# likojack/bnv_fusion

Hardware: AMD Instinct MI355X
Metric: depth frames/sec fused+decoded, 640x480 @ 256^3 grid (higher is better)
Workload: dtype f32 operands split into f16 hi+lo, 3 products on v_mfma_f32_16x16x32_f16, f32 accumulate

## Files before the change

### bnv_fusion_amd/csrc/encode_mlp.hip

```cpp
#include "encode.hpp"

namespace bnv {

__device__ __forceinline__ f32x16 relu16(f32x16 v) {
#pragma unroll
  for (int r = 0; r < 16; ++r) v[r] = relu_bits(v[r]);
  return v;
}

__device__ __forceinline__ f32x16 bias_init(const float* __restrict__ b, int mb, int h) {
  f32x16 v;
#pragma unroll
  for (int q = 0; q < 4; ++q) {
    const f32x4 t = *(const f32x4*)&b[mb * 32 + 8 * q + 4 * h];
#pragma unroll
    for (int i = 0; i < 4; ++i) v[4 * q + i] = t[i];
  }
  return v;
}

__device__ __forceinline__ void layer128(const float* __restrict__ wp, const float* __restrict__ bias,
                                         const f32x16 (&in)[4], f32x16 (&out)[4], int lane, int h) {
#pragma unroll
  for (int mb = 0; mb < 4; ++mb) out[mb] = bias_init(bias, mb, h);
#pragma unroll
  for (int nb = 0; nb < 4; ++nb) {
#pragma unroll
    for (int rq = 0; rq < 4; ++rq) {
      f32x4 a[4];
#pragma unroll
      for (int mb = 0; mb < 4; ++mb)
        a[mb] = *(const f32x4*)&wp[(((mb * 4 + nb) * 4 + rq) * 64 + lane) * 4];
#pragma unroll
      for (int i = 0; i < 4; ++i) {
#pragma unroll
        for (int mb = 0; mb < 4; ++mb)
          out[mb] = __builtin_amdgcn_mfma_f32_32x32x2f32(a[mb][i], in[nb][4 * rq + i], out[mb], 0, 0, 0);
      }
    }
  }
}

__global__ __launch_bounds__(512, 2) void k_pointnet_scatter(
    const float* __restrict__ pts, int n_points, bnv_grid_t g, const float* __restrict__ wpack,
    const uint32_t* __restrict__ bitmap, const uint32_t* __restrict__ word_prefix,
    int32_t* __restrict__ counts, long long* __restrict__ acc, const int32_t* __restrict__ pair_list,
    const int32_t* __restrict__ n_pairs) {
  extern __shared__ __attribute__((aligned(16))) float lds[];
  stage_to_lds<512>(wpack, lds, PN_TOTAL * 4);
  __syncthreads();

  const int lane = threadIdx.x & 63;
  const int wave = __builtin_amdgcn_readfirstlane(threadIdx.x >> 6);
  const int j = lane & 31, h = lane >> 5;
  const PairTiles T = pair_tiles(n_points, pair_list, n_pairs);
  const int n_tiles = T.n_tiles;

  for (int t = blockIdx.x * 8 + wave; t < n_tiles; t += gridDim.x * 8) {
    int i = 0, k = 0;
    const bool have = tile_pair(T, t, j, &i, &k);
    float in0 = 0.f, in1 = 0.f, in2 = 0.f;
    int slot = -1;
    bool valid = false;
    if (have) {
      const float* p = pts + (size_t)i * 6;
      const float x = p[0], y = p[1], z = p[2];
      valid = in_bounds(x, y, z, g);
      if (valid) {
        const float xn = voxel_coord(x, g.bound_min[0], g.voxel_size);
        const float yn = voxel_coord(y, g.bound_min[1], g.voxel_size);
        const float zn = voxel_coord(z, g.bound_min[2], g.voxel_size);
        int gx, gy, gz;
        const uint32_t id = corner_voxel(k, xn, yn, zn, g, gx, gy, gz);
        if (voxel_owner(gx, gy, gz, g) == g.shard_rank) slot = slot_rank(bitmap[id >> 5], word_prefix[id >> 5], id);
        const float rx = relative_coord(xn, gx, g.voxel_size);
        const float ry = relative_coord(yn, gy, g.voxel_size);
        const float rz = relative_coord(zn, gz, g.voxel_size);
        in0 = h ? ry : rx;
        in1 = h ? p[3] : rz;
        in2 = h ? p[5] : p[4];
      }
    }
    if (__ballot(slot >= 0) == 0ULL) continue;

    f32x16 ha[4], hb[4];
#pragma unroll
    for (int mb = 0; mb < 4; ++mb) ha[mb] = bias_init(lds + PN_B1, mb, h);
    {
      const float bin[3] = {in0, in1, in2};
#pragma unroll
      for (int s = 0; s < 3; ++s) {
#pragma unroll
        for (int mb = 0; mb < 4; ++mb)
          ha[mb] = __builtin_amdgcn_mfma_f32_32x32x2f32(lds[PN_W1 + (s * 4 + mb) * 64 + lane], bin[s],
                                                        ha[mb], 0, 0, 0);
      }
    }
#pragma unroll
    for (int mb = 0; mb < 4; ++mb) ha[mb] = relu16(ha[mb]);
    layer128(lds + PN_W2, lds + PN_B2, ha, hb, lane, h);
#pragma unroll
    for (int mb = 0; mb < 4; ++mb) hb[mb] = relu16(hb[mb]);
    layer128(lds + PN_W3, lds + PN_B3, hb, ha, lane, h);
#pragma unroll
    for (int mb = 0; mb < 4; ++mb) ha[mb] = relu16(ha[mb]);
    f32x16 o;
#pragma unroll
    for (int r = 0; r < 16; ++r) o[r] = 0.f;
    {
      const f32x4 b4 = *(const f32x4*)&lds[PN_B4 + 4 * h];
#pragma unroll
      for (int r = 0; r < 4; ++r) o[r] = b4[r];
    }
#pragma unroll
    for (int nb = 0; nb < 4; ++nb) {
#pragma unroll
      for (int rq = 0; rq < 4; ++rq) {
        f32x4 a = {0.f, 0.f, 0.f, 0.f};
        if (j < 8) a = *(const f32x4*)&lds[PN_W4 + ((((nb * 4 + rq) * 2 + h) * 8) + j) * 4];
#pragma unroll
        for (int i = 0; i < 4; ++i)
          o = __builtin_amdgcn_mfma_f32_32x32x2f32(a[i], ha[nb][4 * rq + i], o, 0, 0, 0);
      }
    }
    scatter_tile(o, slot, j, h, counts, acc);
  }
}

typedef __attribute__((address_space(3))) const half8 lds_half8_t;
typedef __attribute__((address_space(3))) const f32x4 lds_f32x4_t;
constexpr int kLdsWin = 61440;

#ifdef BNV_PHASE_PROF
__device__ unsigned long long g_enc_phase[8 * 16];
#define BNV_EPH(i)                                                                          \
  do {                                                                                      \
    if ((threadIdx.x & 63) == 0) {                                                          \
      unsigned long long* _p = (unsigned long long*)((char*)lds + PX_LDS_BYTES) + (threadIdx.x >> 6) * 16; \
      const unsigned long long _t = clock64();                                              \
      _p[i] += _t - _p[15];                                                                 \
      _p[15] = _t;                                                                          \
    }                                                                                       \
  } while (0)
constexpr int kEncProfLds = 8 * 16 * 8;
#else
#define BNV_EPH(i)
constexpr int kEncProfLds = 0;
#endif

struct EncLdsX {
  uint32_t w[3];
  uint32_t b;
};
__device__ __forceinline__ half8 ldsx_wfrag(const EncLdsX& L, int byte_off) {
  const int b = byte_off / kLdsWin;
  return *(lds_half8_t*)((b == 0 ? L.w[0] : (b == 1 ? L.w[1] : L.w[2])) + (uint32_t)(byte_off - b * kLdsWin));
}
__device__ __forceinline__ f32x4 ldsx_bias(const EncLdsX& L, int layer, int rb) {
  return *(lds_f32x4_t*)(L.b + (uint32_t)((layer * 128 + rb * 16) * 4));
}

template <int NPROD>
__device__ __forceinline__ void layer128_x(const EncLdsX& L, int w_off, int layer, const half8 (&inh)[4][2],
                                           const half8 (&inl)[4][2], f32x4 (&out)[8][2]) {
#pragma unroll
  for (int rb = 0; rb < 8; ++rb) out[rb][0] = out[rb][1] = ldsx_bias(L, layer, rb);
  half8 ah[2], al[2];
#define BNV_LOAD_WX(q)                                                        \
  {                                                                           \
    const int wb = (w_off + (q) * 2 * 64 * 8) * 2;                            \
    ah[(q) & 1] = ldsx_wfrag(L, wb);                                          \
    if (NPROD == 3) al[(q) & 1] = ldsx_wfrag(L, wb + 1024);                   \
  }
  BNV_LOAD_WX(0);
#pragma unroll
  for (int q = 0; q < 32; ++q) {
    if (q + 1 < 32) BNV_LOAD_WX(q + 1);
    __builtin_amdgcn_sched_barrier(0);
    const int s = q >> 3, rb = q & 7;
    if constexpr (NPROD == 3) {
      out[rb][0] = __builtin_amdgcn_mfma_f32_16x16x32_f16(al[q & 1], inh[s][0], out[rb][0], 0, 0, 0);
      out[rb][1] = __builtin_amdgcn_mfma_f32_16x16x32_f16(al[q & 1], inh[s][1], out[rb][1], 0, 0, 0);
      out[rb][0] = __builtin_amdgcn_mfma_f32_16x16x32_f16(ah[q & 1], inl[s][0], out[rb][0], 0, 0, 0);
      out[rb][1] = __builtin_amdgcn_mfma_f32_16x16x32_f16(ah[q & 1], inl[s][1], out[rb][1], 0, 0, 0);
    }
    out[rb][0] = __builtin_amdgcn_mfma_f32_16x16x32_f16(ah[q & 1], inh[s][0], out[rb][0], 0, 0, 0);
    out[rb][1] = __builtin_amdgcn_mfma_f32_16x16x32_f16(ah[q & 1], inh[s][1], out[rb][1], 0, 0, 0);
    __builtin_amdgcn_sched_barrier(0);
  }
#undef BNV_LOAD_WX
}

template <int NPROD>
__device__ __forceinline__ void split_x(const f32x4 (&acc)[8][2], half8 (&oh)[4][2], half8 (&ol)[4][2]) {
#pragma unroll
  for (int s = 0; s < 4; ++s)
#pragma unroll
    for (int cb = 0; cb < 2; ++cb) {
      float x[8];
#pragma unroll
      for (int e = 0; e < 8; ++e) x[e] = relu_bits(acc[2 * s + (e >> 2)][cb][e & 3]);
      if (NPROD == 3) {
        split8_f16(x, oh[s][cb], ol[s][cb]);
      } else {
#pragma unroll
        for (int e = 0; e < 8; ++e) oh[s][cb][e] = (_Float16)x[e];
      }
    }
}

__device__ __forceinline__ void scatter_tile_x(const f32x4& o, int slot, int n, int g, int32_t* __restrict__ counts,
                                               long long* __restrict__ acc) {
  uint32_t lo[4], hi[4];
#pragma unroll
  for (int q = 0; q < 4; ++q) fixed_hi_lo(o[q], hi[q], lo[q]);
  asm volatile(BNV_SCAN_ROWS : BNV_SCAN_REGS(lo, hi) : : "vcc");
  {
    const int tsrc = ((g & 1) * 16 + 15) * 4;
#pragma unroll
    for (int q = 0; q < 4; ++q) {
      const uint32_t tl = (uint32_t)__builtin_amdgcn_ds_bpermute(tsrc, (int)lo[q]);
      const uint32_t th = (uint32_t)__builtin_amdgcn_ds_bpermute(tsrc, (int)hi[q]);
      if (g >= 2) {
        const unsigned long long v = (((unsigned long long)hi[q] << 32) | lo[q]) + (((unsigned long long)th << 32) | tl);
        lo[q] = (uint32_t)v;
        hi[q] = (uint32_t)(v >> 32);
      }
    }
  }
  const int p = (g >> 1) * 16 + n;
  const int slot15 = __builtin_amdgcn_readlane(slot, 15);
  const int prev_row = __builtin_amdgcn_update_dpp(0, slot, 0x111 , 0xf, 0xf, false);
  const int prev = n == 0 ? slot15 : prev_row;
  const unsigned long long heads64 = __ballot(p == 0 || prev != slot);
  const uint32_t heads = ((uint32_t)heads64 & 0xffffu) | (((uint32_t)(heads64 >> 32) & 0xffffu) << 16);
  const int s = 31 - __clz((int)(heads & (0xffffffffu >> (31 - p))));
  const bool is_end = p == 31 || ((heads >> (p + 1)) & 1u);
  const int sp = s > 0 ? s - 1 : 0;
  const int src = (((sp >> 4) * 2 + (g & 1)) * 16 + (sp & 15)) * 4;
  uint32_t plo[4], phi[4];
#pragma unroll
  for (int q = 0; q < 4; ++q) {
    plo[q] = (uint32_t)__builtin_amdgcn_ds_bpermute(src, (int)lo[q]);
    phi[q] = (uint32_t)__builtin_amdgcn_ds_bpermute(src, (int)hi[q]);
  }
#ifdef BNV_PROBE_NO_SCATTER
  if ((blockIdx.x & 63) != 0) return;
#endif
  if (slot >= 0 && is_end) {
    unsigned long long* dst = (unsigned long long*)acc + ((uint32_t)slot * 8u + 4u * (uint32_t)(g & 1));
#pragma unroll
    for (int q = 0; q < 4; ++q) {
      unsigned long long v = ((unsigned long long)hi[q] << 32) | lo[q];
      if (s > 0) v -= ((unsigned long long)phi[q] << 32) | plo[q];
      atomicAdd(dst + q, v);
    }
    if ((g & 1) == 0) atomicAdd(&counts[slot], p - s + 1);
  }
}

template <int NPROD>
__global__ __launch_bounds__(512, 2) __attribute__((amdgpu_num_vgpr(120))) void k_pointnet_scatter_x(
    const float* __restrict__ pts, int n_points, bnv_grid_t g, const float* __restrict__ wpack,
    const uint32_t* __restrict__ bitmap, const uint32_t* __restrict__ word_prefix,
    int32_t* __restrict__ counts, long long* __restrict__ acc, int32_t* __restrict__ error,
    const int32_t* __restrict__ pair_list, const int32_t* __restrict__ n_pairs) {
  extern __shared__ __attribute__((aligned(16))) float lds[];
  const float n_cert = wpack[PN_CERT];
  float* lb = lds + PX_TOTAL / 2;
  for (int i = threadIdx.x; i < 128 * 3 + 8; i += 512) lb[i] = wpack[PN_B1 + i];
  stage_to_lds<512>(wpack + PX_OFF, lds, PX_TOTAL * 2);
  int* tile_ctr = (int*)((char*)lds + PX_TOTAL * 2 + (128 * 3 + 8) * 4);
  if (threadIdx.x == 0) *tile_ctr = 0;
  __syncthreads();

  const int lane = threadIdx.x & 63;
  const int n = lane & 15, gk = lane >> 4;
  const int pair = (gk >> 1) * 16 + n;
  const PairTiles T = pair_tiles(n_points, pair_list, n_pairs);
  const int n_tiles = T.n_tiles;
  const int nyz = g.n_xyz[1] * g.n_xyz[2];
  EncLdsX L;
  {
    const uint32_t lds0 = (uint32_t)(uintptr_t)(__attribute__((address_space(3))) float*)lds;
    L.w[0] = lds0 + lane * 16;
    L.w[1] = L.w[0] + kLdsWin;
    L.w[2] = L.w[0] + 2 * kLdsWin;
    L.b = lds0 + PX_TOTAL * 2 + gk * 16;
    asm volatile("" : "+v"(L.w[0]), "+v"(L.w[1]), "+v"(L.w[2]), "+v"(L.b));
  }

  const int tstep = gridDim.x * 8;
  auto grab = [&]() -> int {
    int c = 0;
    if (lane == 0) c = atomicAdd(tile_ctr, 1);
    c = __builtin_amdgcn_readfirstlane(c);
    return blockIdx.x * 8 + (c & 7) + (c >> 3) * tstep;
  };
  float raw[6];
  int raw_k = 0;
  bool raw_ok = false;
  float nin[6];
  uint32_t n_id = 0, n_word = 0, n_pref = 0;
  bool n_own = false;
  auto stage1 = [&](int t) {
    raw_ok = false;
    if (t < n_tiles) {
      int i = 0;
      if (tile_pair(T, t, pair, &i, &raw_k)) {
        const float* p = pts + (size_t)i * 6;
#pragma unroll
        for (int c = 0; c < 6; ++c) raw[c] = p[c];
        raw_ok = true;
      }
    }
  };
  auto stage2 = [&](int t) {
    n_own = false;
#pragma unroll
    for (int c = 0; c < 6; ++c) nin[c] = 0.f;
    if (raw_ok && in_bounds(raw[0], raw[1], raw[2], g)) {
      const int k = raw_k;
      const float xn = voxel_coord(raw[0], g.bound_min[0], g.voxel_size);
      const float yn = voxel_coord(raw[1], g.bound_min[1], g.voxel_size);
      const float zn = voxel_coord(raw[2], g.bound_min[2], g.voxel_size);
      int gx, gy, gz;
      corner_xyz(k, xn, yn, zn, gx, gy, gz);
      if (voxel_owner(gx, gy, gz, g) == g.shard_rank) {
        n_own = true;
        n_id = voxel_id(gx, gy, gz, nyz, g.n_xyz[2]);
        n_word = bitmap[n_id >> 5];
        n_pref = word_prefix[n_id >> 5];
      }
      if ((gk & 1) == 0) {
        nin[0] = relative_coord(xn, gx, g.voxel_size);
        nin[1] = relative_coord(yn, gy, g.voxel_size);
        nin[2] = relative_coord(zn, gz, g.voxel_size);
        nin[3] = raw[3];
        nin[4] = raw[4];
        nin[5] = raw[5];
      }
      if (!(fmaxf(fmaxf(fabsf(raw[3]), fabsf(raw[4])), fabsf(raw[5])) <= n_cert)) *error = 3;
    }
  };
  int t = grab();
  stage1(t);
  stage2(t);
  int t_next = grab(), t_next2 = 0;
  stage1(t_next);
#ifdef BNV_PHASE_PROF
  if ((threadIdx.x & 63) < 16)
    ((unsigned long long*)((char*)lds + PX_LDS_BYTES))[(threadIdx.x >> 6) * 16 + (threadIdx.x & 63)] = 0;
  if ((threadIdx.x & 63) == 0) ((unsigned long long*)((char*)lds + PX_LDS_BYTES))[(threadIdx.x >> 6) * 16 + 15] = clock64();
#endif

  for (; t < n_tiles; t = t_next, t_next = t_next2) {
    float in[6];
#pragma unroll
    for (int c = 0; c < 6; ++c) in[c] = nin[c];
    const int slot = n_own ? slot_rank(n_word, n_pref, n_id) : -1;
    stage2(t_next);
    t_next2 = grab();
    stage1(t_next2);
    __builtin_amdgcn_sched_barrier(0);
    BNV_EPH(0);
    if (__ballot(slot >= 0) == 0ULL) continue;

    f32x4 ha[8][2], hb[8][2];
    {
      half8 bh[2], bl[2];
#pragma unroll
      for (int cb = 0; cb < 2; ++cb) {
        float x[8];
#pragma unroll
        for (int e = 0; e < 8; ++e) x[e] = 0.f;
#pragma unroll
        for (int e = 0; e < 6; ++e) {
          const float other = __shfl(in[e], (lane + 32) & 63, 64);
          x[e] = gk == 0 ? (cb == 0 ? in[e] : other) : 0.f;
        }
        if (NPROD == 3) {
          split8_f16(x, bh[cb], bl[cb]);
        } else {
#pragma unroll
          for (int e = 0; e < 8; ++e) bh[cb][e] = (_Float16)x[e];
        }
      }
#pragma unroll
      for (int rb = 0; rb < 8; ++rb) {
        const half8 ahi = ldsx_wfrag(L, (PX_W1 + rb * 2 * 64 * 8) * 2), alo = ldsx_wfrag(L, (PX_W1 + rb * 2 * 64 * 8) * 2 + 1024);
        const f32x4 b = ldsx_bias(L, 0, rb);
#pragma unroll
        for (int cb = 0; cb < 2; ++cb) {
          f32x4 c = b;
          if constexpr (NPROD == 3) {
            c = __builtin_amdgcn_mfma_f32_16x16x32_f16(alo, bh[cb], c, 0, 0, 0);
            c = __builtin_amdgcn_mfma_f32_16x16x32_f16(ahi, bl[cb], c, 0, 0, 0);
          }
          ha[rb][cb] = __builtin_amdgcn_mfma_f32_16x16x32_f16(ahi, bh[cb], c, 0, 0, 0);
        }
      }
    }
    BNV_EPH(1);
    half8 sh[4][2], sl[4][2];
    split_x<NPROD>(ha, sh, sl);
    BNV_EPH(2);
    layer128_x<NPROD>(L, PX_W2, 1, sh, sl, hb);
    BNV_EPH(3);
    split_x<NPROD>(hb, sh, sl);
    BNV_EPH(4);
    layer128_x<NPROD>(L, PX_W3, 2, sh, sl, ha);
    BNV_EPH(5);
    split_x<NPROD>(ha, sh, sl);
    BNV_EPH(6);
    f32x4 o[2];
    o[0] = o[1] = *(lds_f32x4_t*)(L.b + 384 * 4);
    {
      half8 w4h[4], w4l[4];
      __builtin_amdgcn_sched_barrier(0);
#pragma unroll
      for (int s = 0; s < 4; ++s) {
        w4h[s] = ldsx_wfrag(L, (PX_W4 + s * 2 * 64 * 8) * 2);
        if (NPROD == 3) w4l[s] = ldsx_wfrag(L, (PX_W4 + s * 2 * 64 * 8) * 2 + 1024);
      }
#pragma unroll
      for (int s = 0; s < 4; ++s) {
#pragma unroll
        for (int cb = 0; cb < 2; ++cb) {
          if constexpr (NPROD == 3) {
            o[cb] = __builtin_amdgcn_mfma_f32_16x16x32_f16(w4l[s], sh[s][cb], o[cb], 0, 0, 0);
            o[cb] = __builtin_amdgcn_mfma_f32_16x16x32_f16(w4h[s], sl[s][cb], o[cb], 0, 0, 0);
          }
          o[cb] = __builtin_amdgcn_mfma_f32_16x16x32_f16(w4h[s], sh[s][cb], o[cb], 0, 0, 0);
        }
      }
    }
    f32x4 mine;
#pragma unroll
    for (int i = 0; i < 4; ++i) {
      const float other = __shfl(o[1][i], (lane + 32) & 63, 64);
      mine[i] = gk < 2 ? o[0][i] : other;
    }
    BNV_EPH(7);
    scatter_tile_x(mine, slot, n, gk, counts, acc);
    BNV_EPH(8);
  }
#ifdef BNV_PHASE_PROF
  if ((threadIdx.x & 63) < 15)
    atomicAdd(&g_enc_phase[(threadIdx.x >> 6) * 16 + (threadIdx.x & 63)],
              ((unsigned long long*)((char*)lds + PX_LDS_BYTES))[(threadIdx.x >> 6) * 16 + (threadIdx.x & 63)]);
#endif
}

int encode_init() {
  const hipFuncAttribute lds = hipFuncAttributeMaxDynamicSharedMemorySize;
  BNV_HIP_CHECK(hipFuncSetAttribute((const void*)k_pointnet_scatter, lds, PN_TOTAL * 4));
  BNV_HIP_CHECK(hipFuncSetAttribute((const void*)k_pointnet_scatter_x<3>, lds, PX_LDS_BYTES + kEncProfLds));
  BNV_HIP_CHECK(hipFuncSetAttribute((const void*)k_pointnet_scatter_x<1>, lds, PX_LDS_BYTES + kEncProfLds));
  return BNV_OK;
}

void launch_encoder_mlp(int mlp, int grid, const float* pts, int n, const bnv_grid_t& g, const float* pack,
                        const EncodeWs& ws, const int32_t* plist, hipStream_t stream) {
  if (mlp == 1 || mlp == 3)
    hipLaunchKernelGGL(mlp == 1 ? k_pointnet_scatter_x<3> : k_pointnet_scatter_x<1>, dim3(grid), dim3(512),
                       PX_LDS_BYTES + kEncProfLds, stream, pts, n, g, pack, ws.bitmap, ws.word_prefix, ws.counts,
                       ws.acc, &ws.ctl->error, plist, &ws.ctl->n_pairs);
  else
    hipLaunchKernelGGL(k_pointnet_scatter, dim3(grid), dim3(512), PN_TOTAL * 4, stream, pts, n, g, pack, ws.bitmap,
                       ws.word_prefix, ws.counts, ws.acc, plist, &ws.ctl->n_pairs);
}

}

#ifdef BNV_PHASE_PROF
extern "C" int bnv_dev_enc_phase_read(unsigned long long* out128) {
  BNV_HIP_CHECK(hipDeviceSynchronize());
  BNV_HIP_CHECK(hipMemcpyFromSymbol(out128, HIP_SYMBOL(bnv::g_enc_phase), 128 * sizeof(unsigned long long)));
  unsigned long long z[128] = {};
  BNV_HIP_CHECK(hipMemcpyToSymbol(HIP_SYMBOL(bnv::g_enc_phase), z, sizeof(z)));
  return BNV_OK;
}
#endif
```

### bnv_fusion_amd/weights.py

```python
import os

import numpy as np

_HERE = os.path.dirname(os.path.abspath(__file__))
DEFAULT_FP32 = os.path.join(_HERE, "weights", "pointnet_fp32.npz")
DEFAULT_TCNN = os.path.join(_HERE, "weights", "pointnet_tcnn.npz")

BN_EPS = 1e-5


def load_npz(path=DEFAULT_FP32):
    with np.load(path) as z:
        return {k: z[k] for k in z.files}


def _np(v):
    return v.detach().cpu().numpy() if hasattr(v, "detach") else np.asarray(v)


def fold_pointnet(sd):
    out = []
    for i in (1, 2, 3, 4):
        p = "pointnet_backbone."
        W = _np(sd[f"{p}conv{i}.weight"]).astype(np.float64)[:, :, 0]
        b = _np(sd[f"{p}conv{i}.bias"]).astype(np.float64)
        s = _np(sd[f"{p}bn{i}.weight"]).astype(np.float64) / np.sqrt(
            _np(sd[f"{p}bn{i}.running_var"]).astype(np.float64) + BN_EPS)
        Wf = W * s[:, None]
        bf = (b - _np(sd[f"{p}bn{i}.running_mean"]).astype(np.float64)) * s + _np(sd[f"{p}bn{i}.bias"]).astype(
            np.float64)
        out.append((Wf.astype(np.float32), bf.astype(np.float32)))
    return out


F16_MAX = 65504.0


def certified_input_bound(layers, fixed, n_free, limit=0.98 * F16_MAX):
    W0 = np.abs(np.asarray(layers[0][0], dtype=np.float64))
    fixed = np.asarray(fixed, dtype=np.float64)
    k = len(fixed)
    assert W0.shape[1] == k + n_free
    a = W0[:, :k] @ fixed + np.abs(np.asarray(layers[0][1], dtype=np.float64))
    c = W0[:, k:].sum(1)
    best = np.inf
    for i, (W, b) in enumerate(layers):
        if i:
            Wa = np.abs(np.asarray(W, dtype=np.float64))
            a, c = Wa @ a + np.abs(np.asarray(b, dtype=np.float64)), Wa @ c
        if (a >= limit).any():
            return 0.0
        with np.errstate(divide="ignore"):
            best = min(best, float(np.min(np.where(c > 0, (limit - a) / c, np.inf))))
    return best


def pointnet_normal_bound(sd):
    return certified_input_bound(fold_pointnet(sd)[:3], [1.0, 1.0, 1.0], 3)


def sdf_feature_bound(sd):
    layers = [(_np(sd[f"nerf.geo_layer{i}.weight"]), _np(sd[f"nerf.geo_layer{i}.bias"])) for i in range(3)]
    return certified_input_bound(layers, [1.5] * 3 + [1.0] * 6, 8)


def pack_pointnet(sd):
    (W1, b1), (W2, b2), (W3, b3), (W4, b4) = fold_pointnet(sd)
    lane = np.arange(64)
    n, h = lane & 31, lane >> 5
    w1p = np.zeros((3, 4, 64), np.float32)
    for s in range(3):
        for mb in range(4):
            w1p[s, mb] = W1[mb * 32 + n, 2 * s + h]

    def pack128(W):
        o = np.zeros((4, 4, 4, 64, 4), np.float32)
        for mb in range(4):
            for nb in range(4):
                for rq in range(4):
                    for i in range(4):
                        o[mb, nb, rq, :, i] = W[mb * 32 + n, nb * 32 + 8 * rq + i + 4 * h]
        return o

    w4p = np.zeros((4, 4, 2, 8, 4), np.float32)
    for nb in range(4):
        for rq in range(4):
            for hh in range(2):
                for i in range(4):
                    w4p[nb, rq, hh, :, i] = W4[:, nb * 32 + 8 * rq + i + 4 * hh]
    fp32_part = np.concatenate([w1p.ravel(), pack128(W2).ravel(), pack128(W3).ravel(), w4p.ravel(),
                                b1, b2, b3, b4]).astype(np.float32)
    trailer = np.zeros(4, np.float32)
    trailer[0] = min(pointnet_normal_bound(sd), 3.0e38)
    return np.concatenate([fp32_part, _pack_pointnet_split16(W1, W2, W3, W4), trailer])


def split_f16(x):
    x = np.asarray(x, dtype=np.float32)
    hi = x.astype(np.float16)
    lo = (x - hi.astype(np.float32)).astype(np.float16)
    return hi, lo


def _slot_feature(jj, h):
    return 8 * (jj >> 2) + 4 * h + (jj & 3)


def _pack_pointnet_split16(W1, W2, W3, W4):
    lane = np.arange(64)
    m, g = lane & 15, lane >> 4
    jj = np.arange(8)
    W1p = np.zeros((128, 32), np.float32)
    W1p[:, :6] = W1
    w1 = np.zeros((8, 2, 64, 8), np.float16)
    for rb in range(8):
        w1[rb, 0], w1[rb, 1] = split_f16(W1p[(16 * rb + m)[:, None], 8 * g[:, None] + jj[None, :]])

    def kidx(s):
        return 32 * s + 16 * (jj[None, :] >> 2) + 4 * g[:, None] + (jj[None, :] & 3)

    def pack128(W):
        o = np.zeros((4, 8, 2, 64, 8), np.float16)
        for s in range(4):
            for rb in range(8):
                o[s, rb, 0], o[s, rb, 1] = split_f16(W[(16 * rb + m)[:, None], kidx(s)])
        return o

    W4p = np.zeros((16, 128), np.float32)
    W4p[:8] = W4
    w4 = np.zeros((4, 2, 64, 8), np.float16)
    for s in range(4):
        w4[s, 0], w4[s, 1] = split_f16(W4p[m[:, None], kidx(s)])
    halves = np.concatenate([w1.ravel(), pack128(W2).ravel(), pack128(W3).ravel(), w4.ravel()])
    assert halves.size == 77824
    return halves.view(np.float32)


def _pack_split(W, nks, n_blocks=8):
    lane = np.arange(64)
    n, h = lane & 31, lane >> 5
    Wp = np.zeros((32 * n_blocks, 16 * nks), np.float32)
    Wp[:W.shape[0], :W.shape[1]] = W
    jj = np.arange(8)
    o = np.zeros((n_blocks, nks, 2, 64, 8), np.float16)
    for w in range(n_blocks):
        for ks in range(nks):
            v = Wp[(32 * w + n)[:, None], 16 * ks + _slot_feature(jj[None, :], h[:, None])]
            o[w, ks, 0], o[w, ks, 1] = split_f16(v)
    return o.ravel()


def _pack_split16(W, n_steps, first_layer=False):
    lane = np.arange(64)
    m, g = lane & 15, lane >> 4
    jj = np.arange(8)
    Wp = np.zeros((256, 32 * n_steps), np.float32)
    Wp[:W.shape[0], :W.shape[1]] = W
    o = np.zeros((8, 2 * n_steps, 2, 64, 8), np.float16)
    for w in range(8):
        for s in range(n_steps):
            for rb in range(2):
                if first_layer:
                    k = 8 * g[:, None] + jj[None, :]
                else:
                    k = 32 * s + 16 * (jj[None, :] >> 2) + 4 * g[:, None] + (jj[None, :] & 3)
                v = Wp[(32 * w + 16 * rb + m)[:, None], k]
                o[w, 2 * s + rb, 0], o[w, 2 * s + rb, 1] = split_f16(v)
    return o.ravel()


def pack_sdf_mlp_bwd(sd):
    Ws = [_np(sd[f"nerf.geo_layer{i}.weight"]).astype(np.float32) for i in range(4)]
    halves = np.concatenate([_pack_split(Ws[3].T, 16), _pack_split(Ws[2].T, 16), _pack_split(Ws[1].T, 16),
                             _pack_split(Ws[0].T, 16, n_blocks=1)])
    assert halves.size == 409600
    return halves.view(np.float32).copy()


def pack_sdf_mlp(sd):
    lane = np.arange(64)
    n, h = lane & 31, lane >> 5

    def pack(W, nkb):
        K = W.shape[1]
        o = np.zeros((8, nkb, 64, 4), np.float32)
        for w in range(8):
            for kb in range(nkb):
                for i in range(4):
                    k = 8 * kb + 4 * h + i
                    ok = k < K
                    o[w, kb, ok, i] = W[32 * w + n[ok], k[ok]]
        return o.ravel()

    Ws = [_np(sd[f"nerf.geo_layer{i}.weight"]).astype(np.float32) for i in range(4)]
    bs = [_np(sd[f"nerf.geo_layer{i}.bias"]).astype(np.float32) for i in range(4)]
    assert Ws[0].shape == (256, 17) and all(W.shape == (256, 256) for W in Ws[1:])
    wa = _np(sd["nerf.fc_alpha.weight"]).astype(np.float32).reshape(256)
    ba = np.zeros(4, np.float32)
    ba[0] = _np(sd["nerf.fc_alpha.bias"]).reshape(-1)[0]
    ba[1] = min(sdf_feature_bound(sd), 3.0e38)
    fp32_part = np.concatenate([pack(Ws[0], 3), pack(Ws[1], 32), pack(Ws[2], 32), pack(Ws[3], 32),
                                bs[0], bs[1], bs[2], bs[3], wa, ba]).astype(np.float32)

    halves = np.concatenate([_pack_split(Ws[0], 2), _pack_split(Ws[1], 16), _pack_split(Ws[2], 16),
                             _pack_split(Ws[3], 16)])
    assert halves.size == 409600
    halves_x = np.concatenate([_pack_split16(Ws[0], 1, first_layer=True), _pack_split16(Ws[1], 8),
                               _pack_split16(Ws[2], 8), _pack_split16(Ws[3], 8)])
    assert halves_x.size == 409600
    return np.concatenate([fp32_part, halves.view(np.float32), halves_x.view(np.float32)])


def _split_tcnn(params, n_in_padded, width=64, n_hidden=3):
    params = _np(params).astype(np.float32).reshape(-1)
    dims = [n_in_padded] + [width] * n_hidden + [16]
    mats, off = [], 0
    for i in range(len(dims) - 1):
        mats.append(params[off: off + dims[i + 1] * dims[i]].reshape(dims[i + 1], dims[i]))
        off += dims[i + 1] * dims[i]
    assert off == params.size, (off, params.size)
    return mats


def _pack_tcnn(mats):
    lane = np.arange(64)
    n, h = lane & 31, lane >> 5
    jj = np.arange(8)
    sf = _slot_feature(jj[None, :], h[:, None])
    out = []
    W0 = mats[0]
    nks = W0.shape[1] // 16
    o = np.zeros((2, nks, 64, 8), np.float16)
    for mb in range(2):
        for ks in range(nks):
            o[mb, ks] = W0[(mb * 32 + n)[:, None], 16 * ks + sf]
    out.append(o.ravel())
    for W in mats[1:-1]:
        o = np.zeros((2, 4, 64, 8), np.float16)
        for mb in range(2):
            for g in range(4):
                o[mb, g] = W[(mb * 32 + n)[:, None], (g >> 1) * 32 + 16 * (g & 1) + sf]
        out.append(o.ravel())
    Wl = np.zeros((32, 64), np.float32)
    Wl[:16] = mats[-1]
    o = np.zeros((4, 64, 8), np.float16)
    for g in range(4):
        o[g] = Wl[n[:, None], (g >> 1) * 32 + 16 * (g & 1) + sf]
    out.append(o.ravel())
    return np.concatenate(out).view(np.float32)


def pack_pointnet_tcnn(params):
    return _pack_tcnn(_split_tcnn(params, 16))


def pack_sdf_tcnn(params):
    return _pack_tcnn(_split_tcnn(params, 32))


def pack_sdf_tcnn_bwd(params):
    W0, W1, W2, W3 = _split_tcnn(params, 32)
    h16 = lambda W: W.astype(np.float16).astype(np.float32)
    lane = np.arange(64)
    n, h = lane & 31, lane >> 5
    sf = _slot_feature(np.arange(8)[None, :], h[:, None])
    out = []
    for W in (h16(W2).T, h16(W1).T):
        o = np.zeros((2, 4, 64, 8), np.float16)
        for mb in range(2):
            for g in range(4):
                o[mb, g] = W[(mb * 32 + n)[:, None], (g >> 1) * 32 + 16 * (g & 1) + sf]
        out.append(o.ravel())
    Wt = h16(W0).T
    o = np.zeros((4, 64, 8), np.float16)
    for g in range(4):
        o[g] = Wt[n[:, None], (g >> 1) * 32 + 16 * (g & 1) + sf]
    out.append(o.ravel())
    halves = np.concatenate(out).view(np.float32)
    return np.concatenate([halves, h16(W3)[0].astype(np.float32)])
```

Before: 563.3.

## Pack split-f16 products into unused K and M slots for first and last layers

```diff
diff --git a/bnv_fusion_amd/csrc/encode_mlp.hip b/bnv_fusion_amd/csrc/encode_mlp.hip
--- a/bnv_fusion_amd/csrc/encode_mlp.hip
+++ b/bnv_fusion_amd/csrc/encode_mlp.hip
@@ -332,14 +332,12 @@
         n_word = bitmap[n_id >> 5];
         n_pref = word_prefix[n_id >> 5];
       }
-      if ((gk & 1) == 0) {
-        nin[0] = relative_coord(xn, gx, g.voxel_size);
-        nin[1] = relative_coord(yn, gy, g.voxel_size);
-        nin[2] = relative_coord(zn, gz, g.voxel_size);
-        nin[3] = raw[3];
-        nin[4] = raw[4];
-        nin[5] = raw[5];
-      }
+      nin[0] = relative_coord(xn, gx, g.voxel_size);
+      nin[1] = relative_coord(yn, gy, g.voxel_size);
+      nin[2] = relative_coord(zn, gz, g.voxel_size);
+      nin[3] = raw[3];
+      nin[4] = raw[4];
+      nin[5] = raw[5];
       if (!(fmaxf(fmaxf(fabsf(raw[3]), fabsf(raw[4])), fabsf(raw[5])) <= n_cert)) *error = 3;
     }
   };
@@ -368,37 +366,38 @@
 
     f32x4 ha[8][2], hb[8][2];
     {
-      half8 bh[2], bl[2];
+      half8 bx[2];
+      float x[2][8];
+#pragma unroll
+      for (int e = 0; e < 8; ++e) x[0][e] = x[1][e] = 0.f;
+#pragma unroll
+      for (int e = 0; e < 6; ++e) {
+        const float other = __shfl(in[e], lane ^ 32, 64);
+        x[0][e] = gk < 2 ? in[e] : other;
+        x[1][e] = gk < 2 ? other : in[e];
+      }
 #pragma unroll
       for (int cb = 0; cb < 2; ++cb) {
-        float x[8];
-#pragma unroll
-        for (int e = 0; e < 8; ++e) x[e] = 0.f;
-#pragma unroll
-        for (int e = 0; e < 6; ++e) {
-          const float other = __shfl(in[e], (lane + 32) & 63, 64);
-          x[e] = gk == 0 ? (cb == 0 ? in[e] : other) : 0.f;
+        typedef unsigned u32x4_t __attribute__((ext_vector_type(4)));
+        if constexpr (NPROD == 3) {
+          half8 h, l;
+          split8_f16(x[cb], h, l);
+          const u32x4_t hu = __builtin_bit_cast(u32x4_t, h), lu = __builtin_bit_cast(u32x4_t, l);
+          u32x4_t bu;
+#pragma unroll
+          for (int p = 0; p < 4; ++p) bu[p] = gk < 2 ? hu[p] : (gk == 2 ? lu[p] : 0u);
+          bx[cb] = __builtin_bit_cast(half8, bu);
+        } else {
+#pragma unroll
+          for (int e = 0; e < 8; ++e) bx[cb][e] = (_Float16)(gk == 0 ? x[cb][e] : 0.f);
         }
-        if (NPROD == 3) {
-          split8_f16(x, bh[cb], bl[cb]);
-        } else {
-#pragma unroll
-          for (int e = 0; e < 8; ++e) bh[cb][e] = (_Float16)x[e];
-        }
       }
 #pragma unroll
       for (int rb = 0; rb < 8; ++rb) {
-        const half8 ahi = ldsx_wfrag(L, (PX_W1 + rb * 2 * 64 * 8) * 2), alo = ldsx_wfrag(L, (PX_W1 + rb * 2 * 64 * 8) * 2 + 1024);
+        const half8 a = ldsx_wfrag(L, (PX_W1 + rb * 2 * 64 * 8) * 2);
         const f32x4 b = ldsx_bias(L, 0, rb);
 #pragma unroll
-        for (int cb = 0; cb < 2; ++cb) {
-          f32x4 c = b;
-          if constexpr (NPROD == 3) {
-            c = __builtin_amdgcn_mfma_f32_16x16x32_f16(alo, bh[cb], c, 0, 0, 0);
-            c = __builtin_amdgcn_mfma_f32_16x16x32_f16(ahi, bl[cb], c, 0, 0, 0);
-          }
-          ha[rb][cb] = __builtin_amdgcn_mfma_f32_16x16x32_f16(ahi, bh[cb], c, 0, 0, 0);
-        }
+        for (int cb = 0; cb < 2; ++cb) ha[rb][cb] = __builtin_amdgcn_mfma_f32_16x16x32_f16(a, bx[cb], b, 0, 0, 0);
       }
     }
     BNV_EPH(1);
@@ -413,33 +412,40 @@
     BNV_EPH(5);
     split_x<NPROD>(ha, sh, sl);
     BNV_EPH(6);
-    f32x4 o[2];
-    o[0] = o[1] = *(lds_f32x4_t*)(L.b + 384 * 4);
+    f32x4 o[2], ol[2];
     {
-      half8 w4h[4], w4l[4];
+      const f32x4 b4 = *(lds_f32x4_t*)(L.b + 384 * 4);
+#pragma unroll
+      for (int i = 0; i < 4; ++i) {
+        o[0][i] = o[1][i] = gk < 2 ? b4[i] : 0.f;
+        ol[0][i] = ol[1][i] = 0.f;
+      }
+    }
+    {
+      half8 w4[4];
       __builtin_amdgcn_sched_barrier(0);
 #pragma unroll
+      for (int s = 0; s < 4; ++s) w4[s] = ldsx_wfrag(L, (PX_W4 + s * 2 * 64 * 8) * 2);
+#pragma unroll
       for (int s = 0; s < 4; ++s) {
-        w4h[s] = ldsx_wfrag(L, (PX_W4 + s * 2 * 64 * 8) * 2);
-        if (NPROD == 3) w4l[s] = ldsx_wfrag(L, (PX_W4 + s * 2 * 64 * 8) * 2 + 1024);
-      }
-#pragma unroll
-      for (int s = 0; s < 4; ++s) {
 #pragma unroll
         for (int cb = 0; cb < 2; ++cb) {
-          if constexpr (NPROD == 3) {
-            o[cb] = __builtin_amdgcn_mfma_f32_16x16x32_f16(w4l[s], sh[s][cb], o[cb], 0, 0, 0);
-            o[cb] = __builtin_amdgcn_mfma_f32_16x16x32_f16(w4h[s], sl[s][cb], o[cb], 0, 0, 0);
-          }
-          o[cb] = __builtin_amdgcn_mfma_f32_16x16x32_f16(w4h[s], sh[s][cb], o[cb], 0, 0, 0);
+          if constexpr (NPROD == 3) ol[cb] = __builtin_amdgcn_mfma_f32_16x16x32_f16(w4[s], sl[s][cb], ol[cb], 0, 0, 0);
+          o[cb] = __builtin_amdgcn_mfma_f32_16x16x32_f16(w4[s], sh[s][cb], o[cb], 0, 0, 0);
         }
       }
     }
     f32x4 mine;
 #pragma unroll
     for (int i = 0; i < 4; ++i) {
-      const float other = __shfl(o[1][i], (lane + 32) & 63, 64);
-      mine[i] = gk < 2 ? o[0][i] : other;
+      if constexpr (NPROD == 3) {
+        const float top0 = o[0][i] + ol[0][i], top1 = o[1][i] + ol[1][i];
+        const float other = __shfl(gk < 2 ? top1 : o[0][i], lane ^ 32, 64);
+        mine[i] = (gk < 2 ? top0 : o[1][i]) + other;
+      } else {
+        const float other = __shfl(o[1][i], lane ^ 32, 64);
+        mine[i] = gk < 2 ? o[0][i] : other;
+      }
     }
     BNV_EPH(7);
     scatter_tile_x(mine, slot, n, gk, counts, acc);
diff --git a/bnv_fusion_amd/weights.py b/bnv_fusion_amd/weights.py
--- a/bnv_fusion_amd/weights.py
+++ b/bnv_fusion_amd/weights.py
@@ -110,11 +110,12 @@
     lane = np.arange(64)
     m, g = lane & 15, lane >> 4
     jj = np.arange(8)
-    W1p = np.zeros((128, 32), np.float32)
-    W1p[:, :6] = W1
     w1 = np.zeros((8, 2, 64, 8), np.float16)
     for rb in range(8):
-        w1[rb, 0], w1[rb, 1] = split_f16(W1p[(16 * rb + m)[:, None], 8 * g[:, None] + jj[None, :]])
+        hi, lo = split_f16(W1[16 * rb + m])
+        for part, kg in ((hi, 0), (lo, 1), (hi, 2)):
+            w1[rb, 0, g == kg, :6] = part[g == kg]
+        w1[rb, 1, g == 0, :6] = lo[g == 0]
 
     def kidx(s):
         return 32 * s + 16 * (jj[None, :] >> 2) + 4 * g[:, None] + (jj[None, :] & 3)
@@ -130,7 +131,9 @@
     W4p[:8] = W4
     w4 = np.zeros((4, 2, 64, 8), np.float16)
     for s in range(4):
-        w4[s, 0], w4[s, 1] = split_f16(W4p[m[:, None], kidx(s)])
+        hi, lo = split_f16(W4p[(m & 7)[:, None], kidx(s)])
+        w4[s, 0] = np.where((m < 8)[:, None], hi, lo)
+        w4[s, 1] = np.where((m < 8)[:, None], lo, 0)
     halves = np.concatenate([w1.ravel(), pack128(W2).ravel(), pack128(W3).ravel(), w4.ravel()])
     assert halves.size == 77824
     return halves.view(np.float32)
```

Result: slower. 554.4 (-1.6%).
